# EnricoMiccoli/nodal

Measured on AMD Instinct MI355X. Metric: circuits_per_sec, higher is better.
Workload: dtype f64; 1 GPU; cfg3: grid(1000) 1e6 nodes, sparse CSR path; n=999999, nnz=4995995, parallelism=one GPU

## Files before the change

nodal_amd/_ffi.py:

```python

import atexit
import ctypes as C
import os
import weakref

import numpy as np

_HERE = os.path.dirname(os.path.abspath(__file__))
LIB_PATH = os.path.join(_HERE, "libnodal_hip.so")

OK, E_INVALID, E_HIP, E_ZERO_RESISTANCE, E_STAMP_COLLISION, E_SINGULAR, E_NOMEM, \
    E_UNSUPPORTED = range(8)
SPARSE_AUTO, SPARSE_PCG, SPARSE_DENSIFY, SPARSE_LU, SPARSE_DIRECT = range(5)
OPT_FORCE_PIVOTING = 1
OPT_GEPP_PANEL = 2
OPT_EXTRA_STREAMS = 3
OPT_BORROW_TABLE = 4
OPT_TRANSIENT_TAPE = 5

_p = C.POINTER
_i32p, _i64p, _f64p, _u8p = _p(C.c_int32), _p(C.c_int64), _p(C.c_double), _p(C.c_uint8)

SIGNATURES = {
    "nodal_version": (C.c_char_p, []),
    "nodal_create": (C.c_int, [C.c_int, _p(C.c_void_p)]),
    "nodal_destroy": (C.c_int, [C.c_void_p]),
    "nodal_last_error": (C.c_char_p, [C.c_void_p]),
    "nodal_upload_components": (C.c_int, [C.c_void_p, C.c_int64, _u8p, _f64p, _i32p, _i32p,
                                          _i32p, _i32p, _i32p, _i32p, C.c_int32, C.c_int32]),
    "nodal_host_alloc": (C.c_int, [C.c_size_t, _p(C.c_void_p)]),
    "nodal_host_free": (C.c_int, [C.c_void_p]),
    "nodal_upload_values": (C.c_int, [C.c_void_p, C.c_int32, _f64p]),
    "nodal_assemble_symbolic": (C.c_int, [C.c_void_p]),
    "nodal_assemble_numeric": (C.c_int, [C.c_void_p, C.c_int32, _i64p]),
    "nodal_get_sizes": (C.c_int, [C.c_void_p, _i64p, _i64p, _i64p]),
    "nodal_export_csr": (C.c_int, [C.c_void_p, _i32p, _i32p, _f64p, _f64p]),
    "nodal_export_dense": (C.c_int, [C.c_void_p, _f64p, _f64p]),
    "nodal_solve_dense": (C.c_int, [C.c_void_p, _f64p, _i32p]),
    "nodal_solve_sparse": (C.c_int, [C.c_void_p, C.c_int32, _f64p, _i32p, _i32p, _f64p]),
    "nodal_download_x": (C.c_int, [C.c_void_p, _f64p]),
    "nodal_solve_pairs": (C.c_int, [C.c_void_p, C.c_int32, C.c_int32, _i32p, _i32p, _f64p, _i32p]),
    "nodal_solve_sources": (C.c_int, [C.c_void_p, C.c_int32, C.c_int32, C.c_int32, _i64p, _f64p, _f64p, _f64p,
                                      _i32p]),
    "nodal_branches": (C.c_int, [C.c_void_p, _f64p, _f64p, _f64p, _f64p]),
    "nodal_solve_sources_branches": (C.c_int, [C.c_void_p, C.c_int32, C.c_int32, C.c_int32, _i64p, _f64p, _f64p, _f64p,
                                               _i32p, _f64p, _i32p, _f64p, _i32p, _f64p, _i32p, _f64p]),
    "nodal_sensitivities": (C.c_int, [C.c_void_p, C.c_int32, C.c_int32, _i32p, _i32p, _i32p, _f64p, _f64p, _f64p, _f64p,
                                      _i32p]),
    "nodal_gradient": (C.c_int, [C.c_void_p, C.c_int32, C.c_int32, _f64p, _f64p, C.c_int32, _i64p, _f64p, _f64p, _f64p,
                                 _f64p, _i32p]),
    "nodal_transient": (C.c_int, [C.c_void_p, C.c_int32, C.c_int32, C.c_int32, C.c_int64, _i64p, C.c_int32, _i64p, _f64p,
                                  _f64p, C.c_int32, _i32p, _i32p, _f64p, C.c_int32, _f64p, _f64p, _i32p, _f64p, _i32p,
                                  _f64p, _i32p, _i32p]),
    "nodal_transient_rlc": (C.c_int, [C.c_void_p, C.c_int32, C.c_int32, C.c_int32, C.c_int64, _i64p, C.c_int32, _i64p, _f64p,
                                      _f64p, C.c_int32, _i32p, _i32p, _f64p, C.c_int32, _f64p, _f64p, _i32p, _f64p, _i32p,
                                      _f64p, _i32p, _i32p, C.c_int64, _i64p, _f64p, C.c_int32, _i32p, _f64p, _f64p]),
    "nodal_transient_gradient": (C.c_int, [C.c_void_p, C.c_int32, C.c_int32, _i32p, _i32p, _f64p, _f64p, _f64p, _f64p, _f64p,
                                           _f64p, _i32p]),
    "nodal_ac_sweep": (C.c_int, [C.c_void_p, C.c_int32, C.c_int32, _f64p, C.c_int64, _u8p, _f64p, _i32p, _i32p, C.c_int32,
                                 _i64p, _f64p, _f64p, C.c_int32, _i32p, _i32p, _f64p, C.c_int32, _i32p, _f64p, C.c_int32,
                                 _f64p, _f64p, _i32p, _f64p, _i32p]),
    "nodal_ac_noise": (C.c_int, [C.c_void_p, C.c_int32, C.c_int32, _f64p, C.c_int64, _u8p, _f64p, _i32p, _i32p, C.c_double,
                                 C.c_int32, _i32p, _i32p, C.c_int64, _f64p, _f64p, _f64p, _f64p, _f64p, _i32p]),
    "nodal_ac_ports": (C.c_int, [C.c_void_p, C.c_int32, C.c_int32, _f64p, C.c_int64, _u8p, _f64p, _i32p, _i32p, C.c_int32,
                                 _i32p, _i32p, _f64p, _f64p, _i32p, _i32p, _f64p, _i32p, _i64p]),
    "nodal_ac_gradient": (C.c_int, [C.c_void_p, C.c_int32, C.c_int32, _f64p, C.c_int64, _u8p, _f64p, _i32p, _i32p, C.c_int32,
                                    _i64p, _f64p, _f64p, C.c_int32, _i32p, _i32p, _f64p, _f64p, _f64p, _f64p, _f64p,
                                    C.c_int32, _f64p, _f64p, _i32p, _i64p]),
    "nodal_port_matrix": (C.c_int, [C.c_void_p, C.c_int32, C.c_int32, _i32p, _i32p, _f64p, _f64p, _f64p, _i32p]),
    "nodal_residual": (C.c_int, [C.c_void_p, _f64p]),
    "nodal_run": (C.c_int, [C.c_void_p, C.c_int32, C.c_int32, C.c_int32, _i32p]),
    "nodal_run_batch": (C.c_int, [C.c_void_p, C.c_int32, C.c_int32, C.c_int32, _f64p, _i32p]),
    "nodal_batch_x_device": (C.c_int, [C.c_void_p, C.c_void_p, C.c_int64]),
    "nodal_x_device": (C.c_int, [C.c_void_p, C.c_void_p, C.c_int64]),
    "nodal_last_timings": (C.c_int, [C.c_void_p, _f64p]),
    "nodal_last_kernel_stats": (C.c_int, [C.c_void_p, _f64p, _i64p, _f64p]),
    "nodal_last_solve_info": (C.c_int, [C.c_void_p, _i32p, _i32p, _f64p]),
    "nodal_synchronize": (C.c_int, [C.c_void_p]),
    "nodal_set_option": (C.c_int, [C.c_void_p, C.c_int32, C.c_int32]),
    "nodal_debug_gemm": (C.c_int, [C.c_void_p, C.c_int32, C.c_int32, C.c_int32, _f64p, _f64p, _f64p]),
    "nodal_debug_sources_rhs": (C.c_int, [C.c_void_p, C.c_int32, C.c_int32, _i64p, _f64p, _f64p]),
    "nodal_debug_residual": (C.c_int, [C.c_void_p, C.c_int32, C.c_int32, C.c_int32, _f64p, _f64p, _f64p, _f64p]),
    "nodal_debug_direct_apply": (C.c_int, [C.c_void_p, C.c_int32, C.c_int32, _f64p, _f64p, _i64p, _i32p]),
    "nodal_debug_hierarchy_info": (C.c_int, [C.c_void_p, _i32p, _i64p, _f64p]),
    "nodal_debug_hierarchy_array": (C.c_int, [C.c_void_p, C.c_int32, C.c_int32, C.c_void_p, C.c_int64, _i64p]),
}

HIERARCHY_ARRAYS = (("acol", np.int32), ("aval", np.float64), ("avalf", np.float32), ("alen", np.int32),
                    ("dinv", np.float64), ("adcol", np.int16), ("agg", np.int32), ("pcol", np.int32),
                    ("pval", np.float64), ("pvalf", np.float32), ("rcol", np.int32), ("rval", np.float64),
                    ("rvalf", np.float32), ("rlen", np.int32), ("wcol", np.int32), ("wval", np.float32),
                    ("wlen", np.int32), ("p2col", np.int32), ("p2val", np.float32), ("p2len", np.int32),
                    ("d2", np.float32), ("wtstart", np.uint32), ("wtcol", np.int32), ("wtval", np.float32),
                    ("wtsrc", np.int32))
HIERARCHY_INFO = ("n", "ld", "nc", "width", "maxlen", "wfix", "nnz", "rld", "rcap", "wslots", "fold_want", "fold", "d16",
                  "in_tail", "refreshed", "dense_coarsest")

_lib = None
_live = weakref.WeakSet()


@atexit.register
def _close_all():
    _closing[0] = True
    for h in list(_live):
        h.close()


class NodalHipError(RuntimeError):
    def __init__(self, status, message):
        super().__init__(f"libnodal_hip status {status}: {message}")
        self.status = status


def load():
    global _lib
    if _lib is None:
        if not os.path.exists(LIB_PATH):
            raise OSError(
                f"{LIB_PATH} not found: build it with `make` (or "
                "`python -c 'import __graft_entry__ as g; g.build()'`) -- "
                "nodal_amd has no CPU fallback")
        lib = C.CDLL(LIB_PATH)
        for name, (res, args) in SIGNATURES.items():
            fn = getattr(lib, name)
            fn.restype, fn.argtypes = res, args
        _lib = lib
    return _lib


def _ptr(arr, ctype):
    return arr.ctypes.data_as(_p(ctype))


PINNED_MIN_BYTES = 1 << 20
_PINNED_POOL = {}
_PINNED_POOL_BYTES = [0]
_PINNED_POOL_MAX = 1 << 30
_pinned_ok = [None]
_closing = [False]


def _pinned_release(addr, nbytes):
    if _lib is None or _closing[0]:
        return
    if _PINNED_POOL_BYTES[0] + nbytes <= _PINNED_POOL_MAX:
        _PINNED_POOL.setdefault(nbytes, []).append(addr)
        _PINNED_POOL_BYTES[0] += nbytes
    else:
        _lib.nodal_host_free(C.c_void_p(addr))


def host_empty(count, dtype):
    dtype = np.dtype(dtype)
    nbytes = int(count) * dtype.itemsize
    if nbytes < PINNED_MIN_BYTES or _pinned_ok[0] is False:
        return np.empty(count, dtype=dtype)
    try:
        lib = load()
    except OSError:
        _pinned_ok[0] = False
        return np.empty(count, dtype=dtype)
    size = (nbytes + 4095) & ~4095
    free = _PINNED_POOL.get(size)
    if free:
        addr = free.pop()
        _PINNED_POOL_BYTES[0] -= size
    else:
        out = C.c_void_p()
        if lib.nodal_host_alloc(size, C.byref(out)) != OK or not out.value:
            _pinned_ok[0] = False
            return np.empty(count, dtype=dtype)
        _pinned_ok[0] = True
        addr = out.value
    buf = (C.c_char * size).from_address(addr)
    weakref.finalize(buf, _pinned_release, addr, size)
    return np.frombuffer(buf, dtype=dtype, count=count)


class Handle:
# ... 512 lines not shown
```

nodal_amd/csrc/knobs.h:

```cpp
#pragma once
#include <stdint.h>
#include <stdlib.h>

#include <optional>

namespace knob {

struct Present {
    const char *name;
    bool now() const { return getenv(name) != nullptr; }
};
struct OnUnless0 {
    const char *name;
    bool now() const { const char *e = getenv(name); return !(e && atoi(e) == 0); }
};
struct OffUnlessNon0 {
    const char *name;
    bool now() const { const char *e = getenv(name); return e && atoi(e) != 0; }
};
struct OnIfSet0 {
    const char *name;
    bool now() const { const char *e = getenv(name); return e != nullptr && atoi(e) == 0; }
};
struct Level {
// ... 2 lines not shown
        const char *e = getenv(name);
        if (!e) return 0;
        const int v = atoi(e);
        return v > 1 ? v : 1;
    }
};
struct Int {
    const char *name;
    int dflt;
    int now() const { const char *e = getenv(name); return e ? atoi(e) : dflt; }
};
struct Int64 {
    const char *name;
    int64_t dflt;
    int64_t now() const { const char *e = getenv(name); return e ? atoll(e) : dflt; }
};
struct Double {
    const char *name;
    double dflt;
    double now() const { const char *e = getenv(name); return e ? atof(e) : dflt; }
};
struct IntIfSet {
    const char *name;
    std::optional<int> now() const { const char *e = getenv(name); return e ? std::optional<int>(atoi(e)) : std::nullopt; }
};
struct Int64IfSet {
    const char *name;
    std::optional<int64_t> now() const { const char *e = getenv(name); return e ? std::optional<int64_t>(atoll(e)) : std::nullopt; }
};
struct DoubleIfSet {
    const char *name;
    std::optional<double> now() const { const char *e = getenv(name); return e ? std::optional<double>(atof(e)) : std::nullopt; }
};
struct Text {
    const char *name;
    const char *now() const { return getenv(name); }
};

inline constexpr Present TRACE{"NODAL_TRACE"};
inline constexpr Level POISON{"NODAL_POISON"};
inline constexpr Present NOFILL{"NODAL_NOFILL"};
inline constexpr Present NANCHECK{"NODAL_NANCHECK"};
inline constexpr Double WAIT_TIMEOUT_S{"NODAL_WAIT_TIMEOUT_S", 60.0};
inline constexpr Text STREAM_PRIORITY{"NODAL_STREAM_PRIORITY"};
inline constexpr IntIfSet EXTRA_STREAMS{"NODAL_EXTRA_STREAMS"};
inline constexpr IntIfSet HOST_THREADS{"NODAL_HOST_THREADS"};
inline constexpr IntIfSet CSV_CHUNKS{"NODAL_CSV_CHUNKS"};
inline constexpr OnUnless0 FOLD_STREAM{"NODAL_FOLD_STREAM"};
inline constexpr OffUnlessNon0 COUNT_LDS{"NODAL_COUNT_LDS"};
inline constexpr IntIfSet DENSE_BLOCKINV{"NODAL_DENSE_BLOCKINV"};
inline constexpr IntIfSet GJ_SCALAR{"NODAL_GJ_SCALAR"};
inline constexpr OnUnless0 GJ_DPP{"NODAL_GJ_DPP"};
inline constexpr OnUnless0 BI_SYM{"NODAL_BI_SYM"};
inline constexpr OnIfSet0 BI_MASKED{"NODAL_BI_MASKED"};
inline constexpr Int PANEL_CUS{"NODAL_PANEL_CUS", 32};
inline constexpr Int64 BI_UNMASK_ROWS{"NODAL_BI_UNMASK_ROWS", 0};
inline constexpr OnUnless0 BI_EARLY_COPY{"NODAL_BI_EARLY_COPY"};
inline constexpr Int BI_FIRST_BLOCKS{"NODAL_BI_FIRST_BLOCKS", 2};
inline constexpr Text BI_SWITCH{"NODAL_BI_SWITCH"};
inline constexpr Text BI_SWITCH2{"NODAL_BI_SWITCH2"};
inline constexpr Text BI_WIDTH{"NODAL_BI_WIDTH"};
inline constexpr IntIfSet GEPP_PANEL{"NODAL_GEPP_PANEL"};
inline constexpr Int GEPP_MAX{"NODAL_GEPP_MAX", 1280};
inline constexpr Present GEPP_PROBE{"NODAL_GEPP_PROBE"};
inline constexpr Int64IfSet FCG_MAXIT{"NODAL_FCG_MAXIT"};
inline constexpr OnUnless0 FCG_HOST_SUM{"NODAL_FCG_HOST_SUM"};
inline constexpr Double FCG_LOOK{"NODAL_FCG_LOOK", 0.75};
inline constexpr OnUnless0 LOWDEG{"NODAL_LOWDEG"};
inline constexpr IntIfSet LOWDEG_SHARE{"NODAL_LOWDEG_SHARE"};
inline constexpr Int64 LOWDEG_MIN{"NODAL_LOWDEG_MIN", 32};
inline constexpr Present SPARSE_FORCE_DIRECT{"NODAL_SPARSE_FORCE_DIRECT"};
inline constexpr Present SPARSE_CHILD_DIRECT{"NODAL_SPARSE_CHILD_DIRECT"};
inline constexpr OnUnless0 SAGG{"NODAL_SAGG"};
inline constexpr OnUnless0 SA_REUSE{"NODAL_SA_REUSE"};
inline constexpr OnUnless0 SA_FORK{"NODAL_SA_FORK"};
inline constexpr Double SA_SPREAD{"NODAL_SA_SPREAD", 16.0};
inline constexpr Double SA_SHARE{"NODAL_SA_SHARE", 0.9};
inline constexpr IntIfSet SA_MIS{"NODAL_SA_MIS"};
inline constexpr Text SA_OMEGA_P{"NODAL_SA_OMEGA_P"};
inline constexpr Double SA_PADSLACK{"NODAL_SA_PADSLACK", 1.3};
inline constexpr OnUnless0 SA_D16{"NODAL_SA_D16"};
inline constexpr Int SA_GG{"NODAL_SA_GG", 40};
inline constexpr Int64 SA_GCAP{"NODAL_SA_GCAP", 16384};
inline constexpr Int SA_GSEG{"NODAL_SA_GSEG", 4};
inline constexpr Text SA_NU{"NODAL_SA_NU"};
inline constexpr Int SA_KCYCLE{"NODAL_SA_KCYCLE", 1};
inline constexpr Int SA_KLEVELS{"NODAL_SA_KLEVELS", 1};
inline constexpr OnUnless0 SA_KFREEZE{"NODAL_SA_KFREEZE"};
inline constexpr OnUnless0 SA_FUSE_DIR{"NODAL_SA_FUSE_DIR"};
inline constexpr OffUnlessNon0 SA_GRAPH{"NODAL_SA_GRAPH"};
inline constexpr Text SA_FOLD_POST{"NODAL_SA_FOLD_POST"};
inline constexpr OffUnlessNon0 SA_FOLD_CHECK{"NODAL_SA_FOLD_CHECK"};
inline constexpr OnUnless0 SA_FOLD_VISIT{"NODAL_SA_FOLD_VISIT"};
inline constexpr Int64 SA_VISIT_CAP{"NODAL_SA_VISIT_CAP", 16777216};
inline constexpr OffUnlessNon0 SA_VISIT_CHECK{"NODAL_SA_VISIT_CHECK"};
inline constexpr OnUnless0 SA_RESTRICT_B{"NODAL_SA_RESTRICT_B"};
inline constexpr OffUnlessNon0 SA_RESTRICT_CHECK{"NODAL_SA_RESTRICT_CHECK"};
inline constexpr OnUnless0 SA_TAIL_DENSE{"NODAL_SA_TAIL_DENSE"};
inline constexpr OffUnlessNon0 SA_TAIL_CHECK{"NODAL_SA_TAIL_CHECK"};
inline constexpr Int SA_TAIL_NU{"NODAL_SA_TAIL_NU", 3};
inline constexpr Present TAIL_PROBE{"NODAL_TAIL_PROBE"};
inline constexpr IntIfSet AMG_PASSES0{"NODAL_AMG_PASSES0"};
inline constexpr IntIfSet AMG_PASSES1{"NODAL_AMG_PASSES1"};
inline constexpr IntIfSet AMG_SWEEPS0{"NODAL_AMG_SWEEPS0"};
inline constexpr IntIfSet AMG_BLOCK{"NODAL_AMG_BLOCK"};
inline constexpr DoubleIfSet AMG_THETA{"NODAL_AMG_THETA"};
inline constexpr Present AMG_KEEP_DENSE{"NODAL_AMG_KEEP_DENSE"};
inline constexpr Present AMG_NOTAIL{"NODAL_AMG_NOTAIL"};
inline constexpr IntIfSet AMG_KMAX{"NODAL_AMG_KMAX"};
inline constexpr OnUnless0 PAIRS_BLOCK{"NODAL_PAIRS_BLOCK"};
inline constexpr OnUnless0 PAIRS_FUNCTIONAL{"NODAL_PAIRS_FUNCTIONAL"};
inline constexpr Int PAIRS_DIRECT{"NODAL_PAIRS_DIRECT", -1};
inline constexpr Int64 PAIRS_DIRECT_MIN{"NODAL_PAIRS_DIRECT_MIN", 256};
inline constexpr Double MULTI_BAR{"NODAL_MULTI_BAR", 1e-14};
inline constexpr IntIfSet PRESOLVE{"NODAL_PRESOLVE"};
inline constexpr OnUnless0 PRESOLVE_KEEP{"NODAL_PRESOLVE_KEEP"};
inline constexpr IntIfSet FGMRES_WINDOW{"NODAL_FGMRES_WINDOW"};
inline constexpr Text DIRECT_NB{"NODAL_DIRECT_NB"};
inline constexpr Int DIRECT_LANES{"NODAL_DIRECT_LANES", 4};
inline constexpr DoubleIfSet DIRECT_MAX_GB{"NODAL_DIRECT_MAX_GB"};
inline constexpr IntIfSet DIRECT_BIG_DIM{"NODAL_DIRECT_BIG_DIM"};
inline constexpr OnUnless0 DIRECT_FRONT_LDS{"NODAL_DIRECT_FRONT_LDS"};
inline constexpr Int DIRECT_LDS_BS{"NODAL_DIRECT_LDS_BS", 64};
inline constexpr OnUnless0 DIRECT_PANEL_REGS{"NODAL_DIRECT_PANEL_REGS"};
inline constexpr OnUnless0 DIRECT_BATCHED{"NODAL_DIRECT_BATCHED"};
inline constexpr OnUnless0 DIRECT_WAVE{"NODAL_DIRECT_WAVE"};
inline constexpr Present DIRECT_LEVELS{"NODAL_DIRECT_LEVELS"};
inline constexpr OnUnless0 DIRECT_SUPER{"NODAL_DIRECT_SUPER"};
inline constexpr OnUnless0 DIRECT_APPLY_STEPPED{"NODAL_DIRECT_APPLY_STEPPED"};
inline constexpr OnUnless0 DIRECT_PEEL{"NODAL_DIRECT_PEEL"};
inline constexpr Int ND_DEPTH{"NODAL_ND_DEPTH", 4};
inline constexpr Int64 ND_PAR{"NODAL_ND_PAR", 20000};
inline constexpr Present SLU_DEBUG{"SLU_DEBUG"};

}
```

nodal_amd/csrc/sagg.hip:

```cpp
#include <hip/hip_ext.h>

#include <atomic>
#include <type_traits>

#include "group.h"

int grounded_flags(nodal_ctx *h, uint8_t *flags_dev);

namespace {

using grp::TB;
constexpr int PW = 4;
constexpr int ACAP = 64;
constexpr int RCAP = 96;
constexpr int RCAP_SMALL = 512;
constexpr int RCAP_SMALL_ROWS = 16384;
inline int rcap_for(int64_t nc) { return nc <= RCAP_SMALL_ROWS ? RCAP_SMALL : RCAP; }
constexpr int W0_MAX = 32;
constexpr int COARSEST = 64;
constexpr int MAX_LEVELS = 12;
constexpr int MIS_ROUNDS = 6;
constexpr int TAIL_MAX_N = 1024;
constexpr int TAIL_LEVELS = 6;
constexpr int TAIL_LDS_BUDGET = 150 * 1024;
constexpr int APAD = 32;
constexpr int DOT_BLOCKS = 1024;
#ifndef NODAL_SA_OMEGA
#define NODAL_SA_OMEGA 0.85
#endif
constexpr double OMEGA = NODAL_SA_OMEGA;
constexpr double OMEGA_P = 0.70;
constexpr double OMEGA_P_COARSE = 0.85;
using cyc_t = nodal_cyc_t;

inline unsigned grid_for(int64_t n, unsigned cap = 8192) {
    int64_t g = (n + TB - 1) / TB;
    if (g < 1) g = 1;
    if (g >= 64) g = (g + 7) & ~(int64_t)7;
    return (unsigned)(g > cap ? cap : g);
}
inline int64_t pad64(int64_t n) { return (n + 63) & ~(int64_t)63; }
inline size_t align256(size_t x) { return (x + 255) & ~(size_t)255; }

__device__ __forceinline__ unsigned xcd_block() {
    const unsigned g = gridDim.x, b = blockIdx.x;
    return (g & 7u) ? b : (b & 7u) * (g >> 3) + (b >> 3);
}


struct Ell {
    int64_t n = 0, ld = 0;
    int32_t width = 0;
    const int32_t *col = nullptr;
    const int16_t *dcol = nullptr;
    const double *val = nullptr;
    const float *valf = nullptr;
    const int32_t *len = nullptr;
};

enum { ST_MAXLEN = 0, ST_GRADED = 1, ST_BADDIAG = 2, ST_OVERFLOW = 3, ST_NNZ = 4, ST_UNASSIGNED = 5,
       ST_MAXR = 6, ST_NC = 7 ,
       ST_FARCOL = 8 ,
       ST_FOLDMISS = 9 ,
       ST_VISITMISS = 10 ,
       ST_RESTRICTMISS = 11 ,
       ST_COUNT = 12 };

struct SLevel {
    int64_t n = 0, ld = 0, nc = 0;
    int32_t width = 0;
    int32_t maxlen = 0;
    int32_t wfix = 0;
    int64_t nnz = 0;
    DevBuf acol, aval, alen, dinv;
    DevBuf adcol;
    bool d16 = false;
    DevBuf agg, pcol, pval;
    DevBuf rcol, rval, rlen;
    int64_t rld = 0;
    DevBuf vec, part, gflag;
    DevBuf avalf, pvalf, rvalf;
    DevBuf wcol, wval, wlen;
    int32_t wslots = 0;
    bool fold_want = false, fold = false;
    DevBuf p2col, p2val, p2len, d2;
    bool visit_want = false, visit = false;
    DevBuf wtstart, wtcol, wtval, wtsrc;
// ... 910 lines not shown
            mine[q] = set[lane * 4 + q];
            cnt += mine[q] >= 0 ? 1 : 0;
        }
        int off = wave_excl_scan(cnt, &total);
        __syncthreads();
#pragma unroll
        for (int q = 0; q < 4; ++q)
            if (mine[q] >= 0) set[off++] = mine[q];
        __syncthreads();
        if (total > ACAP) {
            my_flags |= 1u;
            total = ACAP;
        }
        myJ = lane < total ? set[lane] : 0x7fffffff;
        __syncthreads();
#pragma unroll
        for (int k = 2; k <= 64; k <<= 1) {
#pragma unroll
            for (int j = k >> 1; j > 0; j >>= 1) {
                const int32_t other = __shfl_xor(myJ, j, 64);
                const bool up = (lane & k) == 0, lower = (lane & j) == 0;
                const int32_t lo = myJ < other ? myJ : other, hi = myJ < other ? other : myJ;
                myJ = (lower == up) ? lo : hi;
            }
        }
        }
        const int nseg = min(maxseg, total <= 16 ? 4 : (total <= 32 ? 2 : 1)), segw = 64 / nseg;
        const int seg = lane / segw;
        const int32_t segJ = __shfl(myJ, lane % segw, 64);
        double acc = 0.0;
        for (int g = 0; g < ngroups; ++g) {
            if (ngroups > 1 || NUMERIC)
                np = galerkin_products(ld, apcol, apval, aplen, rld, rcol, rval, I, g * G, min(G, rl - g * G), lJ, lV);
            int chunk = (((np + nseg - 1) / nseg) + 7) & ~7;
            if (nseg > 1 && ((chunk >> 3) & 1) == 0) chunk += 8;
            for (int p = seg * chunk; p < (seg + 1) * chunk; p += 8) {
                int32_t j8[8];
                double v8[8];
#pragma unroll
                for (int u = 0; u < 8; ++u) {
                    j8[u] = lJ[p + u];
                    v8[u] = lV[p + u];
                }
#pragma unroll
                for (int u = 0; u < 8; ++u) acc += j8[u] == segJ ? v8[u] : 0.0;
            }
            __syncthreads();
        }
        if (nseg == 4) {
            const double a1 = __shfl(acc, lane + 16, 64), a2 = __shfl(acc, lane + 32, 64), a3 = __shfl(acc, lane + 48, 64);
            acc = (acc + a1) + (a2 + a3);
        } else if (nseg == 2) {
            acc += __shfl(acc, lane + 32, 64);
        }
        if (lane >= total && lane < APAD) {
            ccol[(int64_t)lane * cld + I] = (int32_t)I;
            cval[(int64_t)lane * cld + I] = 0.0;
            cvalf[(int64_t)lane * cld + I] = 0.0f;
        }
        if (lane < total) {
            ccol[(int64_t)lane * cld + I] = myJ;
            cval[(int64_t)lane * cld + I] = acc;
            cvalf[(int64_t)lane * cld + I] = (float)acc;
            if (myJ == (int32_t)I) {
                if (!(acc > 0.0)) my_flags |= 4u;
                cdinv[I] = acc > 0.0 ? 1.0 / acc : 1.0;
            }
        }
        if (lane == 0) {
            clen[I] = total;
            my_max = (uint32_t)total > my_max ? (uint32_t)total : my_max;
            my_nnz += (uint32_t)total;
        }
        __syncthreads();
    }
    if (lane == 0) {
        bstat[blockIdx.x] = my_max;
        bstat[BSTAT_MAX + blockIdx.x] = my_nnz;
    }
    if (my_flags & 1u) atomicOr(&stats[ST_OVERFLOW], 1ull);
    if (my_flags & 4u) atomicOr(&stats[ST_BADDIAG], 1ull);
}

__global__ __launch_bounds__(256) void coarsest_inverse(Ell A, double *__restrict__ inv,
                                                        unsigned long long *__restrict__ stats) {
    __shared__ double M[COARSEST][2 * COARSEST + 1];
    const int n = (int)A.n;
    for (int t = threadIdx.x; t < n * 2 * n; t += 256) {
        const int r = t / (2 * n), c = t % (2 * n);
        M[r][c] = (c >= n && c - n == r) ? 1.0 : 0.0;
    }
    __syncthreads();
    for (int r = threadIdx.x; r < n; r += 256)
        for (int s = 0; s < A.len[r]; ++s) M[r][A.col[(int64_t)s * A.ld + r]] = A.val[(int64_t)s * A.ld + r];
    __syncthreads();
    for (int k = 0; k < n; ++k) {
        const double pv = M[k][k];
        if (!(pv > 0.0)) {
            if (threadIdx.x == 0) atomicOr(&stats[ST_BADDIAG], 2ull);
            return;
        }
        const double rp = 1.0 / pv;
        __syncthreads();
        for (int c = threadIdx.x; c < 2 * n; c += 256) M[k][c] *= rp;
        __syncthreads();
        for (int t = threadIdx.x; t < n * 2 * n; t += 256) {
            const int r = t / (2 * n), c = t % (2 * n);
            if (r != k && c != k) M[r][c] = fma(-M[r][k], M[k][c], M[r][c]);
        }
        __syncthreads();
        for (int r = threadIdx.x; r < n; r += 256)
            if (r != k) M[r][k] = 0.0;
        __syncthreads();
    }
    for (int t = threadIdx.x; t < n * n; t += 256) inv[t] = M[t / n][n + t % n];
}

__global__ __launch_bounds__(TB) void flags_up(int64_t n, const int32_t *__restrict__ agg,
                                               const uint8_t *__restrict__ fine, uint8_t *__restrict__ coarse) {
    for (int64_t i = (int64_t)xcd_block() * TB + threadIdx.x; i < n; i += (int64_t)gridDim.x * TB)
        if (fine[i]) coarse[agg[i]] = 1;
}
__global__ __launch_bounds__(64) void last_level_floating(Ell A, const uint8_t *__restrict__ grounded,
                                                          uint32_t *__restrict__ floating) {
    __shared__ int label[COARSEST];
    __shared__ int changed;
    const int n = (int)A.n, i = threadIdx.x;
    if (i < n) label[i] = i;
    __syncthreads();
    for (int it = 0; it < COARSEST; ++it) {
        if (i == 0) changed = 0;
        __syncthreads();
        int best = i < n ? label[i] : 0;
        if (i < n)
            for (int s = 0; s < A.len[i]; ++s) {
                const int l = label[A.col[(int64_t)s * A.ld + i]];
                best = l < best ? l : best;
            }
        __syncthreads();
        if (i < n && best < label[i]) {
            label[i] = best;
            changed = 1;
        }
        __syncthreads();
        if (!changed) break;
        __syncthreads();
    }
    __shared__ int ok[COARSEST];
    if (i < n) ok[i] = 0;
    __syncthreads();
    if (i < n && grounded[i]) ok[label[i]] = 1;
    __syncthreads();
    if (i < n && label[i] == i && !ok[i]) *floating = 1;
}

__global__ __launch_bounds__(TB) void any_unflagged(int64_t n, const uint8_t *__restrict__ grounded,
                                                    uint32_t *__restrict__ floating) {
    for (int64_t i = (int64_t)xcd_block() * TB + threadIdx.x; i < n; i += (int64_t)gridDim.x * TB)
        if (!grounded[i]) *floating = 1;
}

}

#include "sagg_cycle.h"

namespace {

constexpr int SAGG_DECLINED = -3;

int width_class(int maxlen) {
    static const int classes[] = {4, 5, 6, 8, 12, 16, 20, 24, 32};
    for (int c : classes)
        if (maxlen <= c) return c;
    return 0;
}
int choose_wfix(int maxlen, int64_t n, int64_t nnz, int pad_limit) {
    const int c = width_class(maxlen);
    if (c == 0 || c > pad_limit) return 0;
    static const double slack = knob::SA_PADSLACK.now();
    if ((double)c * (double)n <= slack * (double)nnz || n <= 32768) return c;
    return 0;
}

SHierarchy *hierarchy_of(nodal_ctx *h) {
    if (!h->sagg) h->sagg = new SHierarchy();
    return static_cast<SHierarchy *>(h->sagg);
}

struct SolveBufs {
    double *r, *p, *p2, *Ap, *part_rz, *part_zap, *part_rr, *part_pap, *sc;
    cyc_t *z, *x0;
    int g0;
};

template <bool NUMERIC>
int galerkin_product(nodal_ctx *h, SHierarchy *H, int l, hipEvent_t r_ready = nullptr, int phase = 0) {
    hipStream_t st = h->stream;
    SLevel *L = H->level(l), *C = H->level(l + 1);
    const int64_t n = L->n, ld = L->ld, nc = C->n;
    Ell A = L->A();
    A.width = L->maxlen;
    unsigned long long *dstats = H->stats.as<unsigned long long>();
    const int apw = A.width <= 6 ? 16 : 64;
    NODAL_HIP_TRY(h, H->apcol.reserve((size_t)apw * ld * 4 + 64));
    NODAL_HIP_TRY(h, H->apval.reserve((size_t)apw * ld * 8 + 64));
    NODAL_HIP_TRY(h, H->aplen.reserve((size_t)ld * 4 + 64));
    int32_t *apcol = H->apcol.as<int32_t>(), *aplen = H->aplen.as<int32_t>();
    double *apval = H->apval.as<double>();
    unsigned long long *lst = dstats + (size_t)l * ST_COUNT;
    const unsigned g = grid_for(n);
    if (phase != 2) {
        const bool w = L->fold_want && L->wslots == apw;
        int32_t *wcol = w ? L->wcol.as<int32_t>() : nullptr, *wlen = w ? L->wlen.as<int32_t>() : nullptr;
        float *wval = w ? L->wval.as<float>() : nullptr;
        const double *dinv = L->dinv.as<double>();
        const int32_t *pc = L->pcol.as<int32_t>();
        const double *pv = L->pval.as<double>();
        const unsigned gl = (unsigned)((n + 63) / 64 < 4096 ? (n + 63) / 64 : 4096);
        if (apw == 16 && w) ap_rows<16, true><<<g, TB, 0, st>>>(A, pc, pv, apcol, apval, aplen, lst, dinv, wcol, wval, wlen);
        else if (apw == 16) ap_rows<16, false><<<g, TB, 0, st>>>(A, pc, pv, apcol, apval, aplen, lst, dinv, wcol, wval, wlen);
        else if (w) ap_rows_lds<64, true><<<gl, 64, 0, st>>>(A, pc, pv, apcol, apval, aplen, lst, dinv, wcol, wval, wlen);
        else ap_rows_lds<64, false><<<gl, 64, 0, st>>>(A, pc, pv, apcol, apval, aplen, lst, dinv, wcol, wval, wlen);
        NODAL_HIP_TRY(h, hipGetLastError());
    }
    if (phase == 1) return NODAL_OK;
    int G = 1024 / apw;
    G = (G < 8 ? 8 : (G > 64 ? 64 : G));
    static const int g_env = knob::SA_GG.now();
    if (g_env >= 8 && g_env <= 64 && apw == 16) G = g_env & ~7;
    const int pcap = G * apw + 72;
    const size_t lds = 1024 + (size_t)pcap * 12;
    static const int64_t gcap = knob::SA_GCAP.now();
    static const int maxseg = knob::SA_GSEG.now();
    const unsigned gg = (unsigned)(nc < gcap ? nc : (gcap < BSTAT_MAX ? gcap : BSTAT_MAX));
    if (r_ready) NODAL_HIP_TRY(h, hipStreamWaitEvent(st, r_ready, 0));
    galerkin<NUMERIC><<<gg, 64, lds, st>>>(
        ld, apcol, apval, aplen, nc, L->rld, L->rcol.as<int32_t>(), L->rval.as<double>(), L->rlen.as<int32_t>(),
        C->ld, C->acol.as<int32_t>(), C->aval.as<double>(), C->avalf.as<float>(), C->alen.as<int32_t>(),
        C->dinv.as<double>(), dstats + (size_t)(l + 1) * ST_COUNT, H->bstat.as<uint32_t>(), G, pcap, maxseg);
    if (!NUMERIC)
        reduce_bstat<<<1, 1024, 0, st>>>((int)gg, H->bstat.as<uint32_t>(), dstats + (size_t)(l + 1) * ST_COUNT,
                                         ST_MAXLEN, ST_NNZ);
    NODAL_HIP_TRY(h, hipGetLastError());
    return NODAL_OK;
}

double omega_p(int level) {
    static double w[2] = {-1.0, -1.0};
    if (w[0] < 0.0) {
        double a = OMEGA_P, b = OMEGA_P_COARSE;
        if (const char *e = knob::SA_OMEGA_P.now()) {
            a = atof(e);
            const char *c = strchr(e, ',');
            b = c ? atof(c + 1) : a;
        }
        w[1] = b > 0.0 && b < 1.2 ? b : OMEGA_P_COARSE;
        w[0] = a > 0.0 && a < 1.0 ? a : OMEGA_P;
    }
    return w[level > 0 ? 1 : 0];
}

constexpr int64_t FOLD_MAX_ROWS = 1 << 19;
struct FoldSetting { int mode = 0; unsigned mask = 0; };
const FoldSetting &fold_setting() {
    static const FoldSetting s = [] {
        FoldSetting f;
        const char *e = knob::SA_FOLD_POST.now();
        if (!e || !*e) return f;
        if (strchr(e, 'l')) {
            f.mode = 3;
            for (const char *q = e; (q = strchr(q, 'l')) != nullptr; ++q) {
                const int k = atoi(q + 1);
                if (q[1] >= '0' && q[1] <= '9' && k < MAX_LEVELS) f.mask |= 1u << k;
            }
        } else {
            f.mode = atoi(e) == 0 ? 1 : 2;
        }
        return f;
    }();
    return s;
}
bool fold_wanted(int level, int64_t n) {
    if (level > 0 && n <= TAIL_MAX_N) return false;
    const FoldSetting &f = fold_setting();
    switch (f.mode) {
    case 1: return false;
    case 2: return true;
    case 3: return (f.mask >> level & 1u) != 0;
    default: return n <= FOLD_MAX_ROWS;
    }
}
void decide_folds(SHierarchy *H, const unsigned long long *hs, bool trace) {
    for (int k = 0; k < H->nlev; ++k) {
        SLevel *L = H->pool[k];
        const bool runs_cycle = k + 1 < H->nlev && (H->tail < 0 || k < H->tail);
        const bool miss = hs[(size_t)k * ST_COUNT + ST_FOLDMISS] != 0;
        L->fold = L->fold_want && runs_cycle && !miss;
        if (trace && L->fold_want && runs_cycle)
            fprintf(stderr, "[sagg] level %d (%lld rows): first post-smoothing sweep %s\n", k, (long long)L->n,
                    miss ? "NOT folded: a row of A P lacks a column of its P row (no stored diagonal)"
                         : "folded into the prolongation");
        const bool wide = hs[(size_t)k * ST_COUNT + ST_VISITMISS] != 0;
        L->visit = L->visit_want && L->fold && !wide;
        if (trace && L->visit_want)
            fprintf(stderr, "[sagg] level %d (%lld rows): visit %s\n", k, (long long)L->n,
                    L->visit ? "in three launches" : "NOT in three launches: W missing, or a row of P2 beyond its slots");
        const unsigned long long over = hs[(size_t)k * ST_COUNT + ST_RESTRICTMISS] |
                                        (H->sym_valid ? H->sym_stats[(size_t)k * ST_COUNT + ST_RESTRICTMISS] : 0ull);
        L->restrict_b = L->restrict_want && L->fold && !L->visit && !over;
        if (trace && L->restrict_want && runs_cycle)
            fprintf(stderr, "[sagg] level %d (%lld rows): restriction %s\n", k, (long long)L->n,
                    L->restrict_b ? "from b beside the residual launch"
                                  : over ? "NOT from b: a row of W^T beyond the per-row sort, or more entries than its arrays hold"
                                         : "NOT from b: W missing, or the level visits in three launches");
    }
}

void apply_nu_knob(SHierarchy *H);
// ... 1785 lines not shown
```

Baseline: 173.7 circuits/s.

## Add sub-wave Galerkin kernel processing four coarse rows per wave

Adds a new Galerkin triple-product kernel that splits each 64-lane wave into four 16-lane groups, each building one coarse row with DPP scans, a small per-group hash table and a rank-based column sort. Rows that exceed the small caps fall back to a full-wave path. It also adds a dynamic product-grouping path for wide AP rows. The goal is to stop a whole wave from being spent on one short coarse row in the AMG setup, at the cost of extra code paths, more divergence and fallback overhead.

```diff
diff --git a/nodal_amd/_ffi.py b/nodal_amd/_ffi.py
--- a/nodal_amd/_ffi.py
+++ b/nodal_amd/_ffi.py
@@ -96,6 +96,12 @@
 HIERARCHY_INFO = ("n", "ld", "nc", "width", "maxlen", "wfix", "nnz", "rld", "rcap", "wslots", "fold_want", "fold", "d16",
                   "in_tail", "refreshed", "dense_coarsest")
 
+GALERKIN_SUB_ROWS = 4
+GALERKIN_SUB_ENTRIES = 32
+GALERKIN_SUB_PRODUCTS = 128
+GALERKIN_SUB_COLUMNS = 16
+GALERKIN_DYN_PRODUCTS = 1024
+
 _lib = None
 _live = weakref.WeakSet()
 
diff --git a/nodal_amd/csrc/galerkin_groups.h b/nodal_amd/csrc/galerkin_groups.h
--- /dev/null
+++ b/nodal_amd/csrc/galerkin_groups.h
@@ -0,0 +1,34 @@
+#pragma once
+
+#if defined(__HIPCC__) || defined(__CUDACC__)
+#define GALERKIN_HD __host__ __device__
+#else
+#define GALERKIN_HD
+#endif
+
+struct GalerkinCaps {
+    int entries;
+    int lanes;
+    int products;
+};
+
+constexpr int GALERKIN_SUB_LANES = 16;
+constexpr int GALERKIN_SUB_ROWS = 4;
+constexpr int GALERKIN_SUB_ENTRIES = 32;
+constexpr int GALERKIN_SUB_PRODUCTS = 128;
+constexpr int GALERKIN_SUB_COLUMNS = 16;
+constexpr int GALERKIN_SUB_STRIDE = GALERKIN_SUB_PRODUCTS + 8;
+
+GALERKIN_HD inline int galerkin_group_candidates(int remaining, const GalerkinCaps &c) {
+    int n = remaining < c.entries ? remaining : c.entries;
+    n = n < c.lanes ? n : c.lanes;
+    return n > 0 ? n : 0;
+}
+
+GALERKIN_HD inline bool galerkin_group_keeps(int k, int candidates, int prefix, const GalerkinCaps &c) {
+    return k < candidates && (k == 0 || prefix <= c.products);
+}
+
+GALERKIN_HD inline int galerkin_sub_entries(int entry_cap) {
+    return entry_cap < GALERKIN_SUB_ENTRIES ? entry_cap : GALERKIN_SUB_ENTRIES;
+}
diff --git a/nodal_amd/csrc/knobs.h b/nodal_amd/csrc/knobs.h
--- a/nodal_amd/csrc/knobs.h
+++ b/nodal_amd/csrc/knobs.h
@@ -108,6 +108,9 @@
 inline constexpr OnUnless0 SA_D16{"NODAL_SA_D16"};
 inline constexpr Int SA_GG{"NODAL_SA_GG", 40};
 inline constexpr Int64 SA_GCAP{"NODAL_SA_GCAP", 16384};
+inline constexpr Int SA_GROWS{"NODAL_SA_GROWS", 4};
+inline constexpr OnUnless0 SA_GDYN{"NODAL_SA_GDYN"};
+inline constexpr Int SA_GLIST{"NODAL_SA_GLIST", 1024};
 inline constexpr Int SA_GSEG{"NODAL_SA_GSEG", 4};
 inline constexpr Text SA_NU{"NODAL_SA_NU"};
 inline constexpr Int SA_KCYCLE{"NODAL_SA_KCYCLE", 1};
diff --git a/nodal_amd/csrc/sagg.hip b/nodal_amd/csrc/sagg.hip
--- a/nodal_amd/csrc/sagg.hip
+++ b/nodal_amd/csrc/sagg.hip
@@ -3,6 +3,7 @@
 #include <atomic>
 #include <type_traits>
 
+#include "galerkin_groups.h"
 #include "group.h"
 
 int grounded_flags(nodal_ctx *h, uint8_t *flags_dev);
@@ -1079,6 +1080,371 @@
     if (my_flags & 4u) atomicOr(&stats[ST_BADDIAG], 1ull);
 }
 
+struct GalerkinArgs {
+    int64_t ld;
+    const int32_t *apcol;
+    const double *apval;
+    const int32_t *aplen;
+    int64_t nc, rld;
+    const int32_t *rcol;
+    const double *rval;
+    const int32_t *rlen;
+    int64_t cld;
+    int32_t *ccol;
+    double *cval;
+    float *cvalf;
+    int32_t *clen;
+    double *cdinv;
+};
+
+template <int CTRL>
+__device__ __forceinline__ int dpp_row(int v) {
+    return __builtin_amdgcn_update_dpp(0, v, CTRL, 0xF, 0xF, true);
+}
+__device__ __forceinline__ int row16_incl_scan(int v) {
+    v += dpp_row<0x111>(v);
+    v += dpp_row<0x112>(v);
+    v += dpp_row<0x114>(v);
+    v += dpp_row<0x118>(v);
+    return v;
+}
+template <int K = 1>
+__device__ __forceinline__ int row16_rank(int32_t v) {
+    int r = dpp_row<0x120 + K>(v) < v ? 1 : 0;
+    if constexpr (K < 15) r += row16_rank<K + 1>(v);
+    return r;
+}
+
+__device__ __forceinline__ int galerkin_products_dyn(const GalerkinArgs &a, int64_t I, int t0, int remaining,
+                                                     const GalerkinCaps &caps, int32_t *lJ, double *lV, int *take) {
+    const int lane = threadIdx.x;
+    const int cand = galerkin_group_candidates(remaining, caps);
+    int32_t i = 0, len = 0;
+    double w = 0.0;
+    if (lane < cand) {
+        const int t = t0 + lane;
+        const int64_t rat = ((int64_t)(t >> 3) * a.rld + I) * 8 + (t & 7);
+        i = a.rcol[rat];
+        w = a.rval[rat];
+        len = a.aplen[i];
+        len = len < 0 ? 0 : (len > caps.products ? caps.products : len);
+    }
+    int all = 0;
+    int o = wave_excl_scan(len, &all);
+    const int tk = __popcll(__ballot(galerkin_group_keeps(lane, cand, o + len, caps)));
+    if (lane >= tk) len = 0;
+    const int np = __shfl(o + len, tk - 1, 64);
+    constexpr int INFL = 8;
+    for (int32_t s0 = 0; s0 < len; s0 += INFL) {
+        int32_t cj[INFL];
+        double cv[INFL];
+#pragma unroll
+        for (int q = 0; q < INFL; ++q) {
+            const int32_t s = s0 + q < len ? s0 + q : s0;
+            cj[q] = a.apcol[(int64_t)s * a.ld + i];
+            cv[q] = a.apval[(int64_t)s * a.ld + i];
+        }
+#pragma unroll
+        for (int q = 0; q < INFL; ++q)
+            if (s0 + q < len) {
+                lJ[o] = cj[q];
+                lV[o] = w * cv[q];
+                ++o;
+            }
+    }
+    for (int p = lane + np; p < np + 72; p += 64) lJ[p] = -1;
+    __syncthreads();
+    *take = tk;
+    return np;
+}
+
+template <bool NUMERIC>
+__device__ __forceinline__ void galerkin_row_wave(const GalerkinArgs &a, int64_t I, const GalerkinCaps &caps, int maxseg,
+                                                  int32_t *set, int32_t *lJ, double *lV, uint32_t &my_max,
+                                                  uint32_t &my_nnz, uint32_t &my_flags) {
+    const int lane = threadIdx.x;
+    const int rl = a.rlen[I];
+    int np = 0, take = 0, ngroups = 0;
+    int total = 0;
+    int32_t myJ = 0x7fffffff;
+    if constexpr (NUMERIC) {
+        total = a.clen[I];
+        if (lane < total) myJ = a.ccol[(int64_t)lane * a.cld + I];
+    } else {
+        for (int k = lane; k < 256; k += 64) set[k] = -1;
+        __syncthreads();
+        for (int t0 = 0; t0 < rl; t0 += take, ++ngroups) {
+            np = galerkin_products_dyn(a, I, t0, rl - t0, caps, lJ, lV, &take);
+            for (int p = lane; p < np; p += 64) {
+                const int32_t J = lJ[p];
+                uint32_t hsh = ((uint32_t)J * 2654435761u) >> 24;
+                for (int probe = 0; probe < 256; ++probe) {
+                    const int32_t old = atomicCAS(&set[hsh], -1, J);
+                    if (old == -1 || old == J) break;
+                    hsh = (hsh + 1) & 255u;
+                    if (probe == 255) my_flags |= 1u;
+                }
+            }
+            __syncthreads();
+        }
+        int32_t mine[4];
+        int cnt = 0;
+#pragma unroll
+        for (int q = 0; q < 4; ++q) {
+            mine[q] = set[lane * 4 + q];
+            cnt += mine[q] >= 0 ? 1 : 0;
+        }
+        int off = wave_excl_scan(cnt, &total);
+        __syncthreads();
+#pragma unroll
+        for (int q = 0; q < 4; ++q)
+            if (mine[q] >= 0) set[off++] = mine[q];
+        __syncthreads();
+        if (total > ACAP) {
+            my_flags |= 1u;
+            total = ACAP;
+        }
+        myJ = lane < total ? set[lane] : 0x7fffffff;
+        __syncthreads();
+#pragma unroll
+        for (int k = 2; k <= 64; k <<= 1) {
+#pragma unroll
+            for (int j = k >> 1; j > 0; j >>= 1) {
+                const int32_t other = __shfl_xor(myJ, j, 64);
+                const bool up = (lane & k) == 0, lower = (lane & j) == 0;
+                const int32_t lo = myJ < other ? myJ : other, hi = myJ < other ? other : myJ;
+                myJ = (lower == up) ? lo : hi;
+            }
+        }
+    }
+    const bool kept = !NUMERIC && ngroups == 1;
+    const int nseg = min(maxseg, total <= 16 ? 4 : (total <= 32 ? 2 : 1)), segw = 64 / nseg;
+    const int seg = lane / segw;
+    const int32_t segJ = __shfl(myJ, lane % segw, 64);
+    double acc = 0.0;
+    for (int t0 = 0; t0 < rl; t0 += take) {
+        if (kept) take = rl;
+        else np = galerkin_products_dyn(a, I, t0, rl - t0, caps, lJ, lV, &take);
+        int chunk = (((np + nseg - 1) / nseg) + 7) & ~7;
+        if (nseg > 1 && ((chunk >> 3) & 1) == 0) chunk += 8;
+        for (int p = seg * chunk; p < (seg + 1) * chunk; p += 8) {
+            int32_t j8[8];
+            double v8[8];
+#pragma unroll
+            for (int u = 0; u < 8; ++u) {
+                j8[u] = lJ[p + u];
+                v8[u] = lV[p + u];
+            }
+#pragma unroll
+            for (int u = 0; u < 8; ++u) acc += j8[u] == segJ ? v8[u] : 0.0;
+        }
+        __syncthreads();
+    }
+    if (nseg == 4) {
+        const double a1 = __shfl(acc, lane + 16, 64), a2 = __shfl(acc, lane + 32, 64), a3 = __shfl(acc, lane + 48, 64);
+        acc = (acc + a1) + (a2 + a3);
+    } else if (nseg == 2) {
+        acc += __shfl(acc, lane + 32, 64);
+    }
+    if (lane >= total && lane < APAD) {
+        a.ccol[(int64_t)lane * a.cld + I] = (int32_t)I;
+        a.cval[(int64_t)lane * a.cld + I] = 0.0;
+        a.cvalf[(int64_t)lane * a.cld + I] = 0.0f;
+    }
+    if (lane < total) {
+        a.ccol[(int64_t)lane * a.cld + I] = myJ;
+        a.cval[(int64_t)lane * a.cld + I] = acc;
+        a.cvalf[(int64_t)lane * a.cld + I] = (float)acc;
+        if (myJ == (int32_t)I) {
+            if (!(acc > 0.0)) my_flags |= 4u;
+            a.cdinv[I] = acc > 0.0 ? 1.0 / acc : 1.0;
+        }
+    }
+    if (lane == 0) {
+        a.clen[I] = total;
+        my_max = (uint32_t)total > my_max ? (uint32_t)total : my_max;
+        my_nnz += (uint32_t)total;
+    }
+    __syncthreads();
+}
+
+template <bool NUMERIC, bool SHARED>
+__global__ __launch_bounds__(64) void galerkin_rows(GalerkinArgs a, unsigned long long *__restrict__ stats,
+                                                    uint32_t *__restrict__ bstat, GalerkinCaps caps, int pcap, int maxseg) {
+    extern __shared__ __attribute__((aligned(16))) char gsm[];
+    int32_t *set = reinterpret_cast<int32_t *>(gsm);
+    double *lV = reinterpret_cast<double *>(gsm + 1024);
+    int32_t *lJ = reinterpret_cast<int32_t *>(lV + pcap);
+    const int lane = threadIdx.x;
+    uint32_t my_max = 0, my_nnz = 0, my_flags = 0;
+    if constexpr (!SHARED) {
+        for (int64_t I = blockIdx.x; I < a.nc; I += gridDim.x)
+            galerkin_row_wave<NUMERIC>(a, I, caps, maxseg, set, lJ, lV, my_max, my_nnz, my_flags);
+    } else {
+        constexpr int32_t NONE = 0x7fffffff;
+        const int sub = lane >> 4, sl = lane & 15;
+        const int ecap = galerkin_sub_entries(caps.entries);
+        int32_t *sJ = lJ + sub * GALERKIN_SUB_STRIDE;
+        double *sV = lV + sub * GALERKIN_SUB_STRIDE;
+        int32_t *tbl = set + sub * GALERKIN_SUB_LANES;
+        const int64_t nq = (a.nc + GALERKIN_SUB_ROWS - 1) / GALERKIN_SUB_ROWS;
+        for (int64_t q = blockIdx.x; q < nq; q += gridDim.x) {
+            const int64_t I = q * GALERKIN_SUB_ROWS + sub;
+            const bool valid = I < a.nc;
+            const int rl = valid ? a.rlen[I] : 0;
+            bool fits = valid && rl <= ecap;
+            int total = 0;
+            int32_t myJ = NONE;
+            if constexpr (NUMERIC) {
+                total = valid ? a.clen[I] : 0;
+                fits = fits && total <= GALERKIN_SUB_COLUMNS;
+                if (fits && sl < total) myJ = a.ccol[(int64_t)sl * a.cld + I];
+            } else {
+                tbl[sl] = -1;
+            }
+            const int t = 2 * sl;
+            int32_t i0 = 0, i1 = 0, len0 = 0, len1 = 0;
+            double w0 = 0.0, w1 = 0.0;
+            if (fits && t < rl) {
+                const int64_t rat = ((int64_t)(t >> 3) * a.rld + I) * 8 + (t & 7);
+                i0 = a.rcol[rat];
+                w0 = a.rval[rat];
+                if (t + 1 < rl) {
+                    i1 = a.rcol[rat + 1];
+                    w1 = a.rval[rat + 1];
+                }
+                len0 = a.aplen[i0];
+                if (t + 1 < rl) len1 = a.aplen[i1];
+                len0 = len0 < 0 ? 0 : (len0 > GALERKIN_SUB_STRIDE ? GALERKIN_SUB_STRIDE : len0);
+                len1 = len1 < 0 ? 0 : (len1 > GALERKIN_SUB_STRIDE ? GALERKIN_SUB_STRIDE : len1);
+            }
+            const int cnt = len0 + len1, incl = row16_incl_scan(cnt);
+            const int np = __shfl(incl, lane | 15, 64);
+            fits = fits && np <= GALERKIN_SUB_PRODUCTS;
+            if (!fits) len0 = len1 = 0;
+            const int o0 = incl - cnt, o1 = o0 + len0;
+            constexpr int INFL = 6;
+            const int lmax = len0 > len1 ? len0 : len1;
+            for (int32_t s0 = 0; s0 < lmax; s0 += INFL) {
+                int32_t cj0[INFL], cj1[INFL];
+                double cv0[INFL], cv1[INFL];
+#pragma unroll
+                for (int u = 0; u < INFL; ++u) {
+                    const int32_t sa = s0 + u < len0 ? s0 + u : 0, sb = s0 + u < len1 ? s0 + u : 0;
+                    cj0[u] = a.apcol[(int64_t)sa * a.ld + i0];
+                    cv0[u] = a.apval[(int64_t)sa * a.ld + i0];
+                    cj1[u] = a.apcol[(int64_t)sb * a.ld + i1];
+                    cv1[u] = a.apval[(int64_t)sb * a.ld + i1];
+                }
+#pragma unroll
+                for (int u = 0; u < INFL; ++u) {
+                    if (s0 + u < len0) {
+                        sJ[o0 + s0 + u] = cj0[u];
+                        sV[o0 + s0 + u] = w0 * cv0[u];
+                    }
+                    if (s0 + u < len1) {
+                        sJ[o1 + s0 + u] = cj1[u];
+                        sV[o1 + s0 + u] = w1 * cv1[u];
+                    }
+                }
+            }
+            const int npf = fits ? np : 0;
+            if (fits && sl < 8) sJ[np + sl] = -1;
+            __syncthreads();
+            if constexpr (!NUMERIC) {
+                bool full = false;
+                for (int p = sl; p < npf; p += GALERKIN_SUB_LANES) {
+                    const int32_t J = sJ[p];
+                    uint32_t hsh = ((uint32_t)J * 2654435761u) >> 28;
+                    for (int probe = 0; probe < GALERKIN_SUB_LANES; ++probe) {
+                        const int32_t old = atomicCAS(&tbl[hsh], -1, J);
+                        if (old == -1 || old == J) break;
+                        hsh = (hsh + 1) & (GALERKIN_SUB_LANES - 1);
+                        if (probe == GALERKIN_SUB_LANES - 1) full = true;
+                    }
+                }
+                __syncthreads();
+                if ((__ballot(full) >> (sub * GALERKIN_SUB_LANES)) & 0xffffull) fits = false;
+                const int32_t c = tbl[sl];
+                myJ = fits && c >= 0 ? c : NONE;
+                total = __popcll((__ballot(myJ != NONE) >> (sub * GALERKIN_SUB_LANES)) & 0xffffull);
+            }
+            const int rank = NUMERIC ? sl : row16_rank(myJ);
+            const int nseg = min(maxseg, 4);
+            int chunk = (((np + nseg - 1) / nseg) + 7) & ~7;
+            if (nseg > 1 && ((chunk >> 3) & 1) == 0) chunk += 8;
+            const int np8 = fits ? (np + 7) & ~7 : 0;
+            double p0 = 0.0, p1 = 0.0, p2 = 0.0, sum = 0.0;
+            int sg = 0, next = chunk;
+            for (int p = 0; p < np8; p += 8) {
+                int32_t j8[8];
+                double v8[8];
+#pragma unroll
+                for (int u = 0; u < 8; ++u) {
+                    j8[u] = sJ[p + u];
+                    v8[u] = sV[p + u];
+                }
+                const bool cut = p == next;
+                p0 = cut && sg == 0 ? sum : p0;
+                p1 = cut && sg == 1 ? sum : p1;
+                p2 = cut && sg == 2 ? sum : p2;
+                sum = cut ? 0.0 : sum;
+                sg += cut ? 1 : 0;
+                next += cut ? chunk : 0;
+#pragma unroll
+                for (int u = 0; u < 8; ++u) sum += j8[u] == myJ ? v8[u] : 0.0;
+            }
+            p0 = sg == 0 ? sum : p0;
+            p1 = sg == 1 ? sum : p1;
+            p2 = sg == 2 ? sum : p2;
+            const double acc = (p0 + p1) + (p2 + (sg == 3 ? sum : 0.0));
+            if (fits) {
+                if (myJ != NONE) {
+                    a.ccol[(int64_t)rank * a.cld + I] = myJ;
+                    a.cval[(int64_t)rank * a.cld + I] = acc;
+                    a.cvalf[(int64_t)rank * a.cld + I] = (float)acc;
+                    if (myJ == (int32_t)I) {
+                        if (!(acc > 0.0)) my_flags |= 4u;
+                        a.cdinv[I] = acc > 0.0 ? 1.0 / acc : 1.0;
+                    }
+                }
+                static_assert(APAD == 2 * GALERKIN_SUB_LANES && GALERKIN_SUB_COLUMNS <= GALERKIN_SUB_LANES, "padding by lane");
+#pragma unroll
+                for (int k = 0; k < 2; ++k) {
+                    const int slot = sl + k * GALERKIN_SUB_LANES;
+                    if (slot >= total) {
+                        a.ccol[(int64_t)slot * a.cld + I] = (int32_t)I;
+                        a.cval[(int64_t)slot * a.cld + I] = 0.0;
+                        a.cvalf[(int64_t)slot * a.cld + I] = 0.0f;
+                    }
+                }
+                if (sl == 0) {
+                    a.clen[I] = total;
+                    my_max = (uint32_t)total > my_max ? (uint32_t)total : my_max;
+                    my_nnz += (uint32_t)total;
+                }
+            }
+            const unsigned long long done = __ballot(fits);
+            __syncthreads();
+            for (int s = 0; s < GALERKIN_SUB_ROWS; ++s) {
+                const int64_t Is = q * GALERKIN_SUB_ROWS + s;
+                if (Is < a.nc && !((done >> (s * GALERKIN_SUB_LANES)) & 1ull))
+                    galerkin_row_wave<NUMERIC>(a, Is, caps, maxseg, set, lJ, lV, my_max, my_nnz, my_flags);
+            }
+        }
+        const uint32_t m1 = __shfl(my_max, 16, 64), m2 = __shfl(my_max, 32, 64), m3 = __shfl(my_max, 48, 64);
+        const uint32_t n1 = __shfl(my_nnz, 16, 64), n2 = __shfl(my_nnz, 32, 64), n3 = __shfl(my_nnz, 48, 64);
+        my_max = max(max(my_max, m1), max(m2, m3));
+        my_nnz += n1 + n2 + n3;
+    }
+    if (lane == 0) {
+        bstat[blockIdx.x] = my_max;
+        bstat[BSTAT_MAX + blockIdx.x] = my_nnz;
+    }
+    if (my_flags & 1u) atomicOr(&stats[ST_OVERFLOW], 1ull);
+    if (my_flags & 4u) atomicOr(&stats[ST_BADDIAG], 1ull);
+}
+
 __global__ __launch_bounds__(256) void coarsest_inverse(Ell A, double *__restrict__ inv,
                                                         unsigned long long *__restrict__ stats) {
     __shared__ double M[COARSEST][2 * COARSEST + 1];
@@ -1231,6 +1597,27 @@
     static const int maxseg = knob::SA_GSEG.now();
     const unsigned gg = (unsigned)(nc < gcap ? nc : (gcap < BSTAT_MAX ? gcap : BSTAT_MAX));
     if (r_ready) NODAL_HIP_TRY(h, hipStreamWaitEvent(st, r_ready, 0));
+    static const bool grows = knob::SA_GROWS.now() != 0, gdyn = knob::SA_GDYN.now();
+    static const int glist = knob::SA_GLIST.now();
+    const bool shared = grows && apw == 16, dyn = gdyn && apw == 64;
+    if (shared || dyn) {
+        GalerkinCaps caps{G, 64, G * apw};
+        if (dyn) caps = GalerkinCaps{64, 64, (glist < apw ? apw : (glist > 1024 ? 1024 : glist)) & ~7};
+        int pc2 = caps.products + 72;
+        if (shared && pc2 < GALERKIN_SUB_ROWS * GALERKIN_SUB_STRIDE) pc2 = GALERKIN_SUB_ROWS * GALERKIN_SUB_STRIDE;
+        const size_t lds2 = 1024 + (size_t)pc2 * 12;
+        const int64_t units = shared ? (nc + GALERKIN_SUB_ROWS - 1) / GALERKIN_SUB_ROWS : nc;
+        const unsigned g2 = (unsigned)(units < (int64_t)gg ? units : (int64_t)gg);
+        const GalerkinArgs ga{ld, apcol, apval, aplen, nc, L->rld, L->rcol.as<int32_t>(), L->rval.as<double>(),
+                              L->rlen.as<int32_t>(), C->ld, C->acol.as<int32_t>(), C->aval.as<double>(),
+                              C->avalf.as<float>(), C->alen.as<int32_t>(), C->dinv.as<double>()};
+        unsigned long long *cst = dstats + (size_t)(l + 1) * ST_COUNT;
+        if (shared) galerkin_rows<NUMERIC, true><<<g2, 64, lds2, st>>>(ga, cst, H->bstat.as<uint32_t>(), caps, pc2, maxseg);
+        else galerkin_rows<NUMERIC, false><<<g2, 64, lds2, st>>>(ga, cst, H->bstat.as<uint32_t>(), caps, pc2, maxseg);
+        if (!NUMERIC) reduce_bstat<<<1, 1024, 0, st>>>((int)g2, H->bstat.as<uint32_t>(), cst, ST_MAXLEN, ST_NNZ);
+        NODAL_HIP_TRY(h, hipGetLastError());
+        return NODAL_OK;
+    }
     galerkin<NUMERIC><<<gg, 64, lds, st>>>(
         ld, apcol, apval, aplen, nc, L->rld, L->rcol.as<int32_t>(), L->rval.as<double>(), L->rlen.as<int32_t>(),
         C->ld, C->acol.as<int32_t>(), C->aval.as<double>(), C->avalf.as<float>(), C->alen.as<int32_t>(),
```

After: 180.1 circuits/s, median of 6. 1.04x the previous value.
